# RyanXLi/OneshotDet

Hardware: AMD Instinct MI355X
Metric: images/sec/GPU fwd+bwd, 800x1024 target + 127x127 query, bs=8; 1->8 GPU scaling (higher is better)
Workload: dtype bf16; 1 GPU; BASELINE.json configs[2]: bs=8/GPU, 800x1024 target + 127x127 query, bf16 MFMA convs, forward (two R-50-FPN backbones, query pooling, correlation, FCOS head, training proposals) + FCOS loss + backward (stem/layer1 frozen) + gradient all-reduce + SGD(momentum) + weight repack; global_batch=8, parallelism=dp1: one rank, no collective anywhere in the step, world_size=1

## Files before the change

### oneshotdet_amd/_lib.py

```python
import ctypes as C
import os

_HERE = os.path.dirname(os.path.abspath(__file__))
LIB_PATH = os.environ.get("OSD_LIB_PATH") or os.path.join(_HERE, "lib", "liboneshotdet_hip.so")

OSD_F32, OSD_BF16 = 0, 1
ABI_VERSION = 4
ACT_NONE, ACT_RELU, ACT_EXP_SCALE = 0, 1, 2
RES_NONE, RES_SAME, RES_UP2X, RES_DOWN2X = 0, 1, 2, 3
GN_SPLITS = 64


class ConvDesc(C.Structure):
    _fields_ = [(n, C.c_int32) for n in (
        "dtype", "n", "h", "w", "cin", "in_stride_n", "in_stride_h", "in_stride_w", "ho", "wo", "cout", "r", "s",
        "stride_h", "stride_w", "pad_h", "pad_w", "w_rows", "out_stride", "res_mode", "res_h", "res_w", "res_stride",
        "act")] + [("act_scale", C.c_float), ("relu_in", C.c_int32), ("algo", C.c_int32), ("reserved0", C.c_int32),
                   ("ordered_ws", C.c_void_p), ("ordered_ws_bytes", C.c_int64)]


_p, _i, _f, _i64 = C.c_void_p, C.c_int, C.c_float, C.c_int64

SIGNATURES = {
    "osd_last_error_string": (C.c_char_p, []),
# ... 79 lines not shown
    "osd_box_decode": (_i, [_p, _p, _p, _p, _p, _p, _p, _i, _i, _i, _i, _p, _f, _f, _p, _f, _i, _p]),
    "osd_append_gt_boxes": (_i, [_p, _p, _p, _p, _p, _p, _p, _p, _i, _i, _i, _p]),
    "osd_proposals_sort_nms": (_i, [_p, _p, _i, _i, _i, _p, _p, _i, _i, _f, _i, _i, _p, _p, _p, _p, _p]),
    "osd_proposals_sort_nms_hint": (_i, [_p, _p, _i, _i, _i, _p, _p, _i, _i, _f, _i, _i, _i, _p, _p, _p, _p, _p, _p]),
    "osd_proposals_workspace_bytes": (_i64, [_i, _i, _i, _i]),
    "osd_box_match_sample": (_i, [_p, _p, _p, _p, _p, _p, _i, _i, _i, _i, _f, _f, _p, _p, _p, _p, _p, _p, _p, _p, _p]),
    "osd_box_loss": (_i, [_p, _p, _p, _p, _i, _i, _i, _f, _f, _p, _p, _i, _i, _p]),
    "osd_voc_match": (_i, [_p, _p, _p, _p, _p, _p, _p, _p, _i, _i, _i, _f, _p, _p, _p]),
    "osd_voc_curves": (_i, [_p, _p, _p, _i, _p, _p, _p]),
    "osd_voc_ap": (_i, [_p, _p, _p, _p, _p, _i, _i, _p, _p]),
    "osd_coco_match": (_i, [_p, _p, _p, _p, _p, _p, _i, _i, _i, _p, _i, _p, _i, _p, _p, _p, _p]),
    "osd_groupnorm_act_rois_bwd": (_i, [_p, _p, _p, _p, _p, _p, _p, _p, _p, _i, _i, _i, _i, _f, _f, _i, _i, _i, _i, _p]),
    "osd_rois_sum": (_i, [_p, _p, _i, _i, _i64, _i, _p]),
    "osd_roi_pool_levels_bwd": (_i, [_i, _p, _p, _p, _p, _p, _p, _p, _i, _i, _i, _i, _i, _i, _i, _p]),
    "osd_image_transform": (_i, [_p, _i, _i, _i, _i, _i, _i, _p, _p, _p, _i, _i, _i, _i, _i, _i, _i, _p, _p]),
    "osd_image_transform_workspace_bytes": (_i64, [_i, _i, _i, _i]),
    "osd_image_transform_batch": (_i, [_i, _p, _p, _p, _p, _p, _p, _i, _p, _p, _p, _i, _i, _i, _i, _i, _i, _i, _p, _p]),
}

BOX_CLS_CE, BOX_CLS_FOCAL, BOX_CLS_MSE = 0, 1, 2
SIGNATURES_BOX_MODES = {
    "osd_box_loss_opt": (_i, [_p, _p, _p, _p, _i, _i, _i, _f, _f, _p, _p, _i, _i, _i, _f, _f, _p]),
    "osd_box_decode_opt": (_i, [_p, _p, _p, _p, _p, _p, _p, _i, _i, _i, _i, _p, _f, _f, _p, _f, _i, _i, _p]),
}

BOX_CLS_L1, BOX_CLS_CXE = 3, 4
SOFT_LABEL_DISCRETE, SOFT_LABEL_LINEAR, SOFT_LABEL_TRANS_LINEAR, SOFT_LABEL_TRANS_4TH_LINEAR = 0, 1, 2, 3
SIGNATURES_SOFT_LABELS = {
    "osd_box_match_sample_soft": (_i, [_p, _p, _p, _p, _p, _p, _i, _i, _i, _i, _f, _f, _p, _p, _p, _p, _p, _p, _p, _p, _i, _p, _p, _p]),
    "osd_box_loss_soft": (_i, [_p, _p, _p, _p, _i, _i, _i, _f, _f, _p, _p, _i, _i, _p, _i, _p]),
}

SIGNATURES_NEG_SUPPORT = {
    "osd_box_loss_neg_support": (_i, [_p, _p, _p, _p, _p, _i, _i, _i, _f, _f, _f, _f, _p, _p, _p, _i, _i, _p]),
}

SIGNATURES_SOLVER = {
    "osd_solver_set": (_i, [_p, _f, _i, _p]),
    "osd_sgd_momentum_multi_dev": (_i, [_p, _p, _i, _p, _p, _p, _p, _f, _p]),
    "osd_sgd_momentum_pack_multi_dev": (_i, [_p, _p, _i, _p, _p, _p, _p, _p, _i, _p, _f, _i, _p]),
}

SIGNATURES_CLASS_SWEEP = {
    "osd_class_sweep_group": (_i, []),
    "osd_correlate_levels_sweep": (_i, [_i, _p, _p, _p, _p, _i, _i, _i, _i, _p]),
    "osd_roi_pool_levels_sweep": (_i, [_i, _p, _p, _p, _p, _p, _p, _p, _i, _i, _i, _i, _i, _i, _i, _p, _i, _p]),
}

SIGNATURES_GALLERY = {
    "osd_correlate_levels_gallery": (_i, [_i, _p, _p, _p, _p, _p, _i, _i, _i, _i, _i, _p]),
    "osd_groupnorm_act_rois_gallery": (_i, [_p, _p, _p, _p, _p, _p, _i, _i, _i, _i, _f, _f, _i, _i, _i, _i, _i, _p]),
}

_lib = None


class OsdError(RuntimeError):
    pass


def load():
    global _lib
    if _lib is not None:
        return _lib
    if not os.path.exists(LIB_PATH):
        raise OsdError("liboneshotdet_hip.so not built (%s missing): run `python -m oneshotdet_amd.build` or "
                       "__graft_entry__.build(); there is no CPU/eager fallback" % LIB_PATH)
    import torch
    lib = C.CDLL(LIB_PATH)
    for name, (res, args) in (list(SIGNATURES.items()) + list(SIGNATURES_BOX_MODES.items()) + list(SIGNATURES_SOFT_LABELS.items())
                              + list(SIGNATURES_NEG_SUPPORT.items()) + list(SIGNATURES_SOLVER.items())
                              + list(SIGNATURES_CLASS_SWEEP.items()) + list(SIGNATURES_GALLERY.items())):
        fn = getattr(lib, name)
        fn.restype = res
        fn.argtypes = args
    if lib.osd_abi_version() != ABI_VERSION:
        raise OsdError("%s reports ABI %d, this binding is written for ABI %d: rebuild it (`python -m oneshotdet_amd.build`)"
                       % (LIB_PATH, lib.osd_abi_version(), ABI_VERSION))
    _lib = lib
    return lib


def check(rc, what=""):
    if rc != 0:
        msg = load().osd_last_error_string()
        err = OsdError("%s failed (%d): %s" % (what, rc, msg.decode() if msg else "?"))
        err.code = rc
        raise err


def call(name, *args):
    lib = load()
    check(getattr(lib, name)(*args), name)
```

### oneshotdet_amd/build.py

```python
import os
import subprocess
import sys

HERE = os.path.dirname(os.path.abspath(__file__))
CSRC = os.path.join(HERE, "csrc")
LIBDIR = os.path.join(HERE, "lib")
TAG = os.environ.get("OSD_BUILD_TAG", "")
LIB = os.path.join(LIBDIR, "liboneshotdet_hip%s.so" % ("_" + TAG if TAG else ""))
SOURCES = ["osd_error.hip", "conv_igemm.hip", "conv_igemm_dma.hip", "conv_igemm_sp.hip", "conv_pred.hip", "conv_px.hip", "conv_wgrad.hip", "conv_wgrad_sk.hip", "backward.hip", "groupnorm_onepass.hip", "loss.hip", "elementwise.hip", "proposals.hip", "box_head.hip", "transforms.hip", "box_train.hip", "evaluation.hip", "query_avgpool.hip", "class_sweep.hip", "gallery.hip"]
HIPCC = os.environ.get("HIPCC", "/opt/rocm/bin/hipcc")
FLAGS = ["--offload-arch=gfx950", "-O3", "-fPIC", "-std=c++17", "-Wno-unused-result"] + os.environ.get("OSD_BUILD_FLAGS", "").split()


def _stale(target, deps):
    if not os.path.exists(target):
        return True
    t = os.path.getmtime(target)
    return any(os.path.getmtime(d) > t for d in deps)


def build_library(force=False, verbose=True):
    os.makedirs(LIBDIR, exist_ok=True)
    objdir = os.path.join(LIBDIR, "obj" + ("_" + TAG if TAG else ""))
    os.makedirs(objdir, exist_ok=True)
    headers = sorted(os.path.join(CSRC, f) for f in os.listdir(CSRC) if f.endswith(".h")) + [os.path.join(os.path.dirname(HERE), "include", h) for h in ("oneshotdet_hip.h", "oneshotdet_hip_box_modes.h", "oneshotdet_hip_soft_labels.h", "oneshotdet_hip_neg_support.h", "oneshotdet_hip_solver.h", "oneshotdet_hip_class_sweep.h", "oneshotdet_hip_gallery.h")]
    keep = set(src.replace(".hip", ".o") for src in SOURCES)
    for f in os.listdir(objdir):
        if f.endswith(".o") and f not in keep:
            os.remove(os.path.join(objdir, f))
    objs, procs = [], []
    for src in SOURCES:
        s = os.path.join(CSRC, src)
        o = os.path.join(objdir, src.replace(".hip", ".o"))
        objs.append(o)
        if force or _stale(o, [s] + headers):
            cmd = [HIPCC] + FLAGS + ["-c", s, "-o", o]
            if verbose:
                print(" ".join(cmd), flush=True)
            procs.append((src, subprocess.Popen(cmd, stdout=subprocess.PIPE, stderr=subprocess.STDOUT)))
    for src, p in procs:
        out, _ = p.communicate()
        if p.returncode != 0:
            sys.stderr.write(out.decode())
            raise RuntimeError("hipcc failed on %s" % src)
    if force or procs or _stale(LIB, objs):
        cmd = [HIPCC, "--offload-arch=gfx950", "-shared", "-fPIC", "-o", LIB] + objs
        if verbose:
            print(" ".join(cmd), flush=True)
        subprocess.check_call(cmd)
    return LIB


if __name__ == "__main__":
    print(build_library(force="--force" in sys.argv))
```

### oneshotdet_amd/ops.py

```python
import ctypes as C
import os

import torch

from . import _lib, spec
from ._lib import (ACT_EXP_SCALE, ACT_NONE, ACT_RELU, GN_SPLITS, OSD_BF16, OSD_F32, RES_DOWN2X, RES_NONE, RES_SAME, RES_UP2X,
                   ConvDesc)

__all__ = ["ACT_NONE", "ACT_RELU", "ACT_EXP_SCALE", "RES_NONE", "RES_SAME", "RES_UP2X", "RES_DOWN2X"]


from . import streams

_stream_handle = streams.raw_handle


def _stream():
    return C.c_void_p(_stream_handle())


from .trace import rec as _rec


def _dt(t):
    if t.dtype == torch.float32:
        return OSD_F32
    if t.dtype == torch.bfloat16:
        return OSD_BF16
    raise TypeError("unsupported activation dtype %s" % t.dtype)


class _Ptr(C.c_void_p):
    """a device address that keeps its tensor alive: `_ptr(x.contiguous())` on a non-contiguous x creates a temporary whose block the
    caching allocator would hand to the NEXT allocation made while the argument list is still being built (before the launch)"""


def _ptr(t):
    if t is None:
        return C.c_void_p(0)
    p = _Ptr(t.data_ptr())
    p.keep = t
    return p


def _chk_dev(*ts):
    for t in ts:
        if t is not None and not t.is_cuda:
            raise _lib.OsdError("oneshotdet_amd ops need device tensors (no CPU path): got %s" % t.device)


def conv_out(n, k, s, p):
    return (n + 2 * p - k) // s + 1


class PackedConv(object):
    __slots__ = ("w", "bias", "cout", "cout_store", "w_rows", "cin_k", "cin_real", "r", "s", "stem")

    def __init__(self, w, bias, cout, cout_store, w_rows, cin_k, r, s, stem=False, cin_real=None):
        self.w, self.bias, self.cout, self.cout_store = w, bias, cout, cout_store
        self.w_rows, self.cin_k, self.r, self.s, self.stem = w_rows, cin_k, r, s, stem
        self.cin_real = cin_k if cin_real is None else cin_real


def _round_up(x, m):
    return (x + m - 1) // m * m


def pack_conv(weight, bias=None, bn=None, dtype=torch.float32, stem=False):
    _chk_dev(weight)
    cout, cin, r, s = weight.shape
    weight = weight.contiguous().float()
    scale = None
    if bn is not None:
        g, b, mean, var = (t.float() for t in bn)
# ... 669 lines not shown


def _wgrad_mode():
    return _stream_handle() in _WGRAD_WS


def conv2d_wgrad(x, dy, dw_packed, r, s, stride, pad, cout, scale=None, db=None, algo=None):
    _chk_dev(x, dy, dw_packed)
    d = _conv_desc(x.shape, _dt(x), cout, r, s, stride, pad, dy.shape[-1])
    assert (dy.shape[1], dy.shape[2]) == (d.ho, d.wo), (dy.shape, d.ho, d.wo)
    st = _stream()

    def launch(dw, dbias):
        _lib.call("osd_conv2d_wgrad", C.byref(d), _p(x), _p(dy), _p(scale), _p(dw), _p(dbias), st)
    key = (d.dtype, tuple(x.shape), cout, r, s, stride, pad, dy.shape[-1], db is not None, _wgrad_mode())
    if algo is None:
        algo = WGRAD_ALGO_CACHE.get(key)
    if algo is None:
        algo = _tune_wgrad(key, d, launch, dw_packed, db, [x.shape[2]]) if _TUNING[0] else 0
    d.algo = algo
    launch(dw_packed, db)
    _rec("wgrad", items=[dict(x=x, dy=dy, dw=dw_packed, scale=scale, db=db, r=r, s=s, stride=stride, pad=pad, cout=cout)], algo=algo, key=key)


PRED_G = 64


def pred_gemm_ok(cout, r, s, stride, pad, cin, n_levels):
    return cout <= 4 and (r, s, stride, pad) == (3, 3, 1, 1) and cin % 256 == 0 and n_levels <= 6


def pred_dy_gather(dys, cout, cin):
    dy0 = dys[0]
    d = _conv_desc((dy0.shape[0], dy0.shape[1], dy0.shape[2], cin), _dt(dy0), cout, 3, 3, 1, 1, dy0.shape[-1])
    k = len(dys)
    tot = sum(t.shape[0] * t.shape[1] * t.shape[2] for t in dys)
    g = torch.empty((tot, PRED_G), device=dy0.device, dtype=dy0.dtype)
    ptrs = (C.c_void_p * k)(*[t.data_ptr() for t in dys])
    ns = (C.c_int32 * k)(*[t.shape[0] for t in dys])
    hs = (C.c_int32 * k)(*[t.shape[1] for t in dys])
    ws = (C.c_int32 * k)(*[t.shape[2] for t in dys])
    _lib.call("osd_pred_dy_gather", C.byref(d), k, ptrs, ns, hs, ws, _p(g), _stream())
    _rec("pred_gather", dys=list(dys), cout=cout, out=g)
    return g


def pred_dgrad_pack(w_master, cout, cin, dtype, out=None):
    wd = torch.empty((cin, 1, 1, PRED_G), device=w_master.device, dtype=dtype) if out is None else out
    _lib.call("osd_pred_dgrad_pack", _dt(wd), _p(w_master), cout, cin, _p(wd), _stream())
    _rec("pred_dgrad_pack", w=w_master, cout=cout, cin=cin, out=wd)
    return wd


def conv2d_wgrad_grouped(pairs, dw_packed, r, s, stride, pad, cout, scale=None, db=None, algo=None, g=None):
    x0, dy0 = pairs[0]
    d = _conv_desc(x0.shape, _dt(x0), cout, r, s, stride, pad, dy0.shape[-1])
    k = len(pairs)
    xs = (C.c_void_p * k)(*[x.data_ptr() for x, _ in pairs])
    dys = (C.c_void_p * k)(*[dy.data_ptr() for _, dy in pairs])
    ns = (C.c_int32 * k)(*[x.shape[0] for x, _ in pairs])
    hs = (C.c_int32 * k)(*[x.shape[1] for x, _ in pairs])
    ws = (C.c_int32 * k)(*[x.shape[2] for x, _ in pairs])
    st = _stream()
    if (cout <= 4 and (r, s, stride, pad) == (3, 3, 1, 1) and x0.shape[-1] % 256 == 0 and scale is None and k <= 6
            and not os.environ.get("OSD_NO_PRED_WGRAD")):
        if g is not None and not os.environ.get("OSD_PRED_WGRAD_READONCE"):
            wsp = torch.empty((64 + PRED_G * x0.shape[-1] + 64,), device=x0.device, dtype=torch.float32)
            _lib.call("osd_conv2d_wgrad_pred_gathered", C.byref(d), k, xs, _p(g), ns, hs, ws, _p(dw_packed), _p(db), _p(wsp), st)
        else:
            need = int(_lib.load().osd_conv2d_wgrad_pred_workspace_bytes(k, ns, hs, ws, x0.shape[-1]))
            wsp = torch.empty((need // 4 + 1,), device=x0.device, dtype=torch.float32)
            _lib.call("osd_conv2d_wgrad_pred", C.byref(d), k, xs, dys, ns, hs, ws, _p(dw_packed), _p(db), _p(wsp), st)
        _rec("wgrad", items=[dict(x=x, dy=dy, dw=dw_packed, scale=None, db=db, r=r, s=s, stride=stride, pad=pad, cout=cout)
                             for x, dy in pairs], algo="pred", key=None)
        return

    def launch(dw, dbias):
        _lib.call("osd_conv2d_wgrad_grouped", C.byref(d), k, xs, dys, ns, hs, ws, _p(scale), _p(dw), _p(dbias), st)
    key = (d.dtype, tuple(tuple(x.shape) for x, _ in pairs), cout, r, s, stride, pad, dy0.shape[-1], db is not None, _wgrad_mode())
    if algo is None:
        algo = WGRAD_ALGO_CACHE.get(key)
    if algo is None:
        algo = _tune_wgrad(key, d, launch, dw_packed, db, [x.shape[2] for x, _ in pairs]) if _TUNING[0] else 0
    d.algo = algo
    launch(dw_packed, db)
    _rec("wgrad", items=[dict(x=x, dy=dy, dw=dw_packed, scale=scale, db=db, r=r, s=s, stride=stride, pad=pad, cout=cout)
                         for x, dy in pairs], algo=algo, key=key)


def conv2d_wgrad_batched(items, r, s, stride, pad, cout, algo=None):
    x0, dy0 = items[0][0], items[0][1]
    assert all(it[0].shape == x0.shape and it[1].shape == dy0.shape for it in items)
    d = _conv_desc(x0.shape, _dt(x0), cout, r, s, stride, pad, dy0.shape[-1])
    k = len(items)
    xs = (C.c_void_p * k)(*[it[0].data_ptr() for it in items])
    dys = (C.c_void_p * k)(*[it[1].data_ptr() for it in items])
    scales = (C.c_void_p * k)(*[(it[3].data_ptr() if it[3] is not None else 0) for it in items])
    st = _stream()
    has_db = any(it[4] is not None for it in items)

    def launch(dws, dbs):
        dwp = (C.c_void_p * k)(*[t.data_ptr() for t in dws])
        dbp = (C.c_void_p * k)(*[(t.data_ptr() if t is not None else 0) for t in dbs])
        _lib.call("osd_conv2d_wgrad_batched", C.byref(d), k, xs, dys, scales, dwp, dbp, st)
    key = ("batched", k, d.dtype, tuple(x0.shape), cout, r, s, stride, pad, dy0.shape[-1], has_db, _wgrad_mode())
    if algo is None:
# ... 569 lines not shown
```

### oneshotdet_amd/train.py

```python
import math
import os

import torch

from . import streams

from . import ops, spec

from .train_backward import BackwardPass
from .train_forward import SIZE_RANGES, ForwardPass
from .train_second_stage import SecondStage
from .train_state import State
from .train_update import Update


def _payload(t):
    from .layers import ImageList
    if isinstance(t, ops.PackedImages):
        return t.tensor
    if isinstance(t, ImageList):
        return t.tensors
    return t


# ... 44 lines not shown
        self.pg = process_group
        self.wstream = torch.cuda.Stream(device=self.device) if wgrad_side_stream else None
        self.s1 = torch.cuda.Stream(device=self.device) if wgrad_side_stream else None
        self.wstream2 = torch.cuda.Stream(device=self.device) if wgrad_side_stream else None
        self.pstream = torch.cuda.Stream(device=self.device) if wgrad_side_stream else None
        self._keep = []
        self.second_stage = bool(second_stage)
        self.box_keys, self.box_losses = None, None
        self.box_suppress_loss = None
        from .model import ProposalDepth
        self._prop_depth = None if os.environ.get("OSD_NO_PROP_HINT") else ProposalDepth()
        self.lockstep = os.environ.get("OSD_LOCKSTEP", "0") != "0"
        self.corr_levels = os.environ.get("OSD_CORR_LEVELS", "1") != "0"
        self.skip_unused_c2 = os.environ.get("OSD_FULL_C2", "0") == "0"
        self.towers_merged = os.environ.get("OSD_TOWERS_MERGED", "0") != "0"
        self.split_levels = os.environ.get("OSD_SPLIT_LEVELS", "0") != "0"
        self.fuse_head_sum = os.environ.get("OSD_NO_HEAD_SUM_FUSION", "0") == "0"
        if not self.siamese_backbone:
            self.BBS = ("backbone.", "backbone.")
        self._shared_held = {}
        sd = {k: torch.as_tensor(v).to(self.device, torch.float32) for k, v in state_dict.items()
              if self.siamese_backbone or not spec.is_query_backbone_key(k)}
        missing = [k for k in spec.hot_path_shapes(self.siamese_backbone) if k not in sd]
        if missing:
            raise KeyError("state_dict is missing hot-path keys (siamese_backbone=%r), e.g. %s" % (self.siamese_backbone, missing[:3]))
        self._frozen_sd = sd
        self.convs = {}
        self.extra = {}
        self._plan = []
        self._build(sd)
        self._allocate(sd)
        from . import model as _model
        self._fused_l1 = {}
        if _model.FUSE_DOWNSAMPLE and dtype == torch.bfloat16:
            for bb in dict.fromkeys(self.BBS):
                if (bb + "body.layer1.0.downsample.0.weight") in sd:
                    self._fused_l1[bb] = _model.pack_conv3_downsample(sd, bb + "body.layer1.0.", dtype)
        from .dist_utils import GradExchange, bucket_ranges
        self.ustream = torch.cuda.Stream(device=self.device)
        for pair in [a for a in os.environ.get("OSD_STREAM_ALIAS", "").split(",") if "=" in a]:
            names = {"w": "wstream", "w2": "wstream2", "s1": "s1", "p": "pstream", "u": "ustream"}
            dst, src = pair.split("=")
            if getattr(self, names[src]) is not None:
                setattr(self, names[dst], getattr(self, names[src]))
        self.exchange = GradExchange(self.flat_g, bucket_ranges(self._plan, self.flat_g.numel()), self.pg,
                                     single_rank_too=exchange_single_rank, wire_dtype=grad_wire_dtype, comm_stream=self.ustream)
        self._overlap, self._fuse_update, self._updated = True, False, set()
        self.consume_grads = os.environ.get("OSD_NO_CONSUME_GRADS", "0") == "0"
        self._grads_clean, self._zeroed = False, set()
        self._wqs = None
        self._pred_grad_bufs = {}
        self.pred_dgrad_gemm = os.environ.get("OSD_NO_PRED_DGRAD_GEMM", "0") == "0"
        self._pred_dgrad = {}
        self.tower_wgrad_at = os.environ.get("OSD_TOWER_WGRAD_AT", "")
        self._held_wgrads = []
        if ordered_wgrad is None:
            ordered_wgrad = os.environ.get("OSD_WGRAD_ORDERED", "0") != "0"
        self.ordered_wgrad = bool(ordered_wgrad)
        self.fuse_gn_bwd = (not self.ordered_wgrad and self.dtype == torch.bfloat16 and os.environ.get("OSD_GN_FUSION", "0") != "0")
        self._gnb_ws = {}
        self.fpn_out_grouped = os.environ.get("OSD_NO_FPN_GROUPED", "0") == "0"
        self.gn_conv_db = (not self.ordered_wgrad and os.environ.get("OSD_NO_GN_CONV_DB", "0") == "0" and not ops.GN_ONEPASS_BWD)
        self.fuse_gn_fwd = (not self.ordered_wgrad and self.dtype == torch.bfloat16 and os.environ.get("OSD_GN_FWD_FUSION", "0") != "0")
        self._gnf_ws = {}
        cands = (self.wstream, self.wstream2) + ((self.pstream,) if self.second_stage else ())
        self._wgrad_streams = list({id(x): x for x in cands if x is not None}.values()) or [streams.current()]
        if self.ordered_wgrad and self.second_stage:
            import warnings
            warnings.warn("ordered_wgrad makes every conv_wgrad launch bit-reproducible, the second stage's included; its "
                          "ROI-pool backward (osd_roi_pool_levels_bwd) still scatters with fp32 atomics, so the gradients it "
                          "feeds into both backbones are reproducible only up to the order of those adds")
        for st in self._wgrad_streams:
            ops.wgrad_set_workspace(st, (1 << 30) if self.ordered_wgrad else 0)
        if self.wstream is not None:
            self.warm_streams()
        self.defer_join = False
        self._deferred, self._defer_now, self._joined_refs = None, False, None
        self.repack()
        self.zero_bias = torch.zeros(4096, device=self.device, dtype=torch.float32)
        weights = [c.w for c in self.convs.values() if c.trainable] + \
                  [p for n, (p, _) in self.extra.items() if "bias" not in n]
        biases = [c.b for c in self.convs.values() if c.trainable and c.has_bias] + \
                 [p for n, (p, _) in self.extra.items() if "bias" in n]
        self.lr, self.momentum, self.weight_decay = lr, momentum, weight_decay
        self.lr_schedule, self._solver, self._dev_update = lr_schedule, None, False
        self.opt = None
        if optimizer == "torch":
            self.opt = torch.optim.SGD([{"params": weights, "lr": lr, "weight_decay": weight_decay},
                                        {"params": biases, "lr": 2 * lr, "weight_decay": 0.0}], lr=lr, momentum=momentum)
            self._sgd = dict(tables={}, buf=None, steps=0)
        else:
            self._build_sgd_table(weights, biases)

    def _add_conv(self, name, sd, bn=None, bias=None, trainable=True):
        w = sd[name + ".weight"]
        cout, cin, r, s = w.shape
        c = TConv(name, cout, cin, r, s, trainable, bias is not None)
        if bn is not None:
            g, b, mean, var = (sd[bn + k] for k in (".weight", ".bias", ".running_mean", ".running_var"))
            c.bn_scale = (g * var.rsqrt()).contiguous()
            c.bn_shift = (b - mean * c.bn_scale).contiguous()
        self.convs[name] = c
        if trainable:
            self._plan.append((name + ".weight", (cout, r, s, cin)))
            if bias is not None:
                self._plan.append((name + ".bias", (cout,)))
# ... 426 lines not shown
```

### oneshotdet_amd/train_backward.py

```python

import torch

from . import streams

from . import ops, spec


class BackwardPass(object):
    def _wstream_of(self, which):
        if self.wstream is None:
            return None
        return self.wstream2 if (which == 1 and self.wstream2 is not None) else self.wstream

    def _on_wstream(self, fn, tensors, which=0):
        ws = self._wstream_of(which)
        if ws is None:
            return fn()
        ev = torch.cuda.Event()
        ev.record()
        ws.wait_event(ev)
        with streams.on(ws):
            fn()
        self._keep.append(tensors)

# ... 4 lines not shown
        ws = self._wstream_of(which)
        producers = [cur if ws is None else ws] + list(extra)
        if self._fuse_update and cur not in producers:
            producers.append(cur)
        if self.exchange.active:
            self.exchange.ready(name, producers)
        if not self._fuse_update:
            return
        ust = self.exchange.comm if self.exchange.active else self.ustream
        if not self.exchange.active:
            for st in producers:
                ev = torch.cuda.Event()
                ev.record(st)
                ust.wait_event(ev)
        with streams.on(ust):
            self._update_bucket(name)

    def _flush_wgrads(self, j, which):
        q, self._wqs[j] = self._wqs[j], []
        for i in range(0, len(q), 24):
            part = q[i:i + 24]
            if len(part) == 1:
                c, x, dy, stride, pad = part[0]
                self._on_wstream(lambda c=c, x=x, dy=dy, stride=stride, pad=pad: ops.conv2d_wgrad(
                    x, dy, c.gw, c.r, c.s, stride, pad, c.cout, scale=c.bn_scale, db=c.gb if c.has_bias else None), (x, dy),
                    which)
            else:
                items = [(x, dy, c.gw, c.bn_scale, c.gb if c.has_bias else None, c.r, c.s, stride, pad, c.cout)
                         for c, x, dy, stride, pad in part]
                self._on_wstream(lambda items=items: ops.conv2d_wgrad_mixed(items), items, which)

    def _flush_shared_stage(self, sname, which0):
        q, self._wqs[0] = self._wqs[0], []
        if which0 == 1:
            ev = torch.cuda.Event()
            ev.record()
            self._shared_held[sname] = (q, ev)
            return False
        held = self._shared_held.pop(sname, None)
        if held is not None:
            ws = self._wstream_of(0) or streams.current()
            ws.wait_event(held[1])
            q = held[0] + q
        self._wqs[0] = q
        self._flush_wgrads(0, 0)
        return True

    def _wgrad_grouped(self, c, pairs, which=0, g=None):
        self._on_wstream(lambda: ops.conv2d_wgrad_grouped(pairs, c.gw, c.r, c.s, 1, c.r // 2, c.cout, scale=c.bn_scale,
                                                          db=c.gb if c.has_bias else None, g=g), (pairs, g), which)

    def _pred_backward(self, c, t_last, dpred, which):
        nl = len(dpred)
        g = ops.pred_dy_gather(dpred, c.cout, c.cin)
        self._wgrad_grouped(c, [(t_last[l], dpred[l]) for l in range(nl)], which, g=g)
        ent = self.pred_dgrad_weights(c, fresh_ok=True)
        dx = ops.conv2d(g.view(1, 1, g.shape[0], ops.PRED_G), ent)
        out, q0 = [], 0
        for t in dpred:
            n, hh, ww = t.shape[0], t.shape[1], t.shape[2]
            out.append(dx.view(-1, c.cin)[q0:q0 + n * hh * ww].view(n, hh, ww, c.cin))
            q0 += n * hh * ww
        return out

    def pred_dgrad_weights(self, c, fresh_ok=False):
        key = ("pred_dgrad", c.name)
        ent = self._pred_dgrad.get(key)
        if ent is None:
            wd = torch.empty((c.cin, 1, 1, ops.PRED_G), device=self.device, dtype=self.dtype)
            ent = self._pred_dgrad[key] = ops.PackedConv(wd, torch.zeros(ops._round_up(c.cin, 16), device=self.device, dtype=torch.float32),
                                                         c.cin, c.cin, c.cin, ops.PRED_G, 1, 1, cin_real=9 * c.cout)
        fresh = getattr(self, "_pred_dgrad_fresh", None)
        if fresh is None:
            fresh = self._pred_dgrad_fresh = set()
        if fresh_ok and c.name in fresh:
            fresh.discard(c.name)
            return ent
        ops.pred_dgrad_pack(c.w, c.cout, c.cin, self.dtype, out=ent.w)
        if not fresh_ok:
            fresh.add(c.name)
        return ent

    def _dgrad_levels(self, c, dys):
        return ops.conv2d_grouped(dys, c.pd, pad=c.r - 1 - (c.r // 2))

    def head_backward(self, feats, ctxs, pred_grads):
        nl = len(feats)
        if self.towers_merged:
            d_t = self._towers_backward(ctxs, pred_grads, self.TOWERS, nl)
        else:
            main = streams.current()
            side = self.s1 if self.s1 is not None else main
            side.wait_stream(main)
            with streams.on(side):
                d_t = self._towers_backward(ctxs, pred_grads, ("bbox_tower",), nl)
            if self.fuse_head_sum:
                def bbox_grads():
                    main.wait_stream(side)
                    self._keep.append(d_t["bbox_tower"])
                    return d_t["bbox_tower"]
                return self._towers_backward(ctxs, pred_grads, ("cls_tower",), nl, last_addends=bbox_grads)["cls_tower"]
            d_t.update(self._towers_backward(ctxs, pred_grads, ("cls_tower",), nl))
            main.wait_stream(side)
        return [ops.add_mask(d_t["cls_tower"][l], d_t["bbox_tower"][l]) for l in range(nl)]

    def _towers_backward(self, ctxs, pred_grads, towers, nl, last_addends=None):
# ... 192 lines not shown
```

Baseline: 784.7 images/sec.

## Fuse prediction-conv dgrad and wgrad into a single gather+MFMA backward kernel

Adds a HIP kernel that gathers the im2col'd dy for the small-cout 3x3 prediction convs once into LDS. It then computes both dx (via packed transposed weights) and per-workgroup partial dw/db with MFMA, followed by a reduction kernel. This replaces the separate dy-gather, grouped wgrad launch and dgrad GEMM, removing repeated reads of dy and x and several launches. The trade-off is that wgrad now runs on the main stream instead of the side wgrad stream, which loses that overlap, and it adds a partial-sum workspace.

```diff
diff --git a/include/oneshotdet_hip_pred_bwd.h b/include/oneshotdet_hip_pred_bwd.h
--- /dev/null
+++ b/include/oneshotdet_hip_pred_bwd.h
@@ -0,0 +1,24 @@
+#ifndef ONESHOTDET_HIP_PRED_BWD_H
+#define ONESHOTDET_HIP_PRED_BWD_H
+
+#include "oneshotdet_hip.h"
+
+#ifdef __cplusplus
+extern "C" {
+#endif
+
+#define OSD_PRED_BWD_BOTH 0
+#define OSD_PRED_BWD_DGRAD 1
+#define OSD_PRED_BWD_WGRAD 2
+
+int64_t osd_pred_bwd_workspace_bytes(int n_seg, const int32_t* ns, const int32_t* hs, const int32_t* ws, int cin, int cout);
+
+int osd_conv2d_pred_bwd(const osd_conv_desc* desc, int n_seg, const void* const* xs, const void* const* dys, const int32_t* ns,
+                        const int32_t* hs, const int32_t* ws, const void* wd_packed, void* dx, float* dw, float* db, void* workspace,
+                        int flags, void* stream);
+
+#ifdef __cplusplus
+}
+#endif
+
+#endif
diff --git a/oneshotdet_amd/_lib.py b/oneshotdet_amd/_lib.py
--- a/oneshotdet_amd/_lib.py
+++ b/oneshotdet_amd/_lib.py
@@ -155,6 +155,12 @@
     "osd_groupnorm_act_rois_gallery": (_i, [_p, _p, _p, _p, _p, _p, _i, _i, _i, _i, _f, _f, _i, _i, _i, _i, _i, _p]),
 }
 
+PRED_BWD_BOTH, PRED_BWD_DGRAD, PRED_BWD_WGRAD = 0, 1, 2
+SIGNATURES_PRED_BWD = {
+    "osd_pred_bwd_workspace_bytes": (_i64, [_i, _p, _p, _p, _i, _i]),
+    "osd_conv2d_pred_bwd": (_i, [C.POINTER(ConvDesc), _i, _p, _p, _p, _p, _p, _p, _p, _p, _p, _p, _i, _p]),
+}
+
 _lib = None
 
 
@@ -173,7 +179,8 @@
     lib = C.CDLL(LIB_PATH)
     for name, (res, args) in (list(SIGNATURES.items()) + list(SIGNATURES_BOX_MODES.items()) + list(SIGNATURES_SOFT_LABELS.items())
                               + list(SIGNATURES_NEG_SUPPORT.items()) + list(SIGNATURES_SOLVER.items())
-                              + list(SIGNATURES_CLASS_SWEEP.items()) + list(SIGNATURES_GALLERY.items())):
+                              + list(SIGNATURES_CLASS_SWEEP.items()) + list(SIGNATURES_GALLERY.items())
+                              + list(SIGNATURES_PRED_BWD.items())):
         fn = getattr(lib, name)
         fn.restype = res
         fn.argtypes = args
diff --git a/oneshotdet_amd/build.py b/oneshotdet_amd/build.py
--- a/oneshotdet_amd/build.py
+++ b/oneshotdet_amd/build.py
@@ -7,7 +7,7 @@
 LIBDIR = os.path.join(HERE, "lib")
 TAG = os.environ.get("OSD_BUILD_TAG", "")
 LIB = os.path.join(LIBDIR, "liboneshotdet_hip%s.so" % ("_" + TAG if TAG else ""))
-SOURCES = ["osd_error.hip", "conv_igemm.hip", "conv_igemm_dma.hip", "conv_igemm_sp.hip", "conv_pred.hip", "conv_px.hip", "conv_wgrad.hip", "conv_wgrad_sk.hip", "backward.hip", "groupnorm_onepass.hip", "loss.hip", "elementwise.hip", "proposals.hip", "box_head.hip", "transforms.hip", "box_train.hip", "evaluation.hip", "query_avgpool.hip", "class_sweep.hip", "gallery.hip"]
+SOURCES = ["osd_error.hip", "conv_igemm.hip", "conv_igemm_dma.hip", "conv_igemm_sp.hip", "conv_pred.hip", "conv_pred_bwd.hip", "conv_px.hip", "conv_wgrad.hip", "conv_wgrad_sk.hip", "backward.hip", "groupnorm_onepass.hip", "loss.hip", "elementwise.hip", "proposals.hip", "box_head.hip", "transforms.hip", "box_train.hip", "evaluation.hip", "query_avgpool.hip", "class_sweep.hip", "gallery.hip"]
 HIPCC = os.environ.get("HIPCC", "/opt/rocm/bin/hipcc")
 FLAGS = ["--offload-arch=gfx950", "-O3", "-fPIC", "-std=c++17", "-Wno-unused-result"] + os.environ.get("OSD_BUILD_FLAGS", "").split()
 
@@ -23,7 +23,7 @@
     os.makedirs(LIBDIR, exist_ok=True)
     objdir = os.path.join(LIBDIR, "obj" + ("_" + TAG if TAG else ""))
     os.makedirs(objdir, exist_ok=True)
-    headers = sorted(os.path.join(CSRC, f) for f in os.listdir(CSRC) if f.endswith(".h")) + [os.path.join(os.path.dirname(HERE), "include", h) for h in ("oneshotdet_hip.h", "oneshotdet_hip_box_modes.h", "oneshotdet_hip_soft_labels.h", "oneshotdet_hip_neg_support.h", "oneshotdet_hip_solver.h", "oneshotdet_hip_class_sweep.h", "oneshotdet_hip_gallery.h")]
+    headers = sorted(os.path.join(CSRC, f) for f in os.listdir(CSRC) if f.endswith(".h")) + [os.path.join(os.path.dirname(HERE), "include", h) for h in ("oneshotdet_hip.h", "oneshotdet_hip_box_modes.h", "oneshotdet_hip_soft_labels.h", "oneshotdet_hip_neg_support.h", "oneshotdet_hip_solver.h", "oneshotdet_hip_class_sweep.h", "oneshotdet_hip_gallery.h", "oneshotdet_hip_pred_bwd.h")]
     keep = set(src.replace(".hip", ".o") for src in SOURCES)
     for f in os.listdir(objdir):
         if f.endswith(".o") and f not in keep:
diff --git a/oneshotdet_amd/csrc/conv_pred_bwd.hip b/oneshotdet_amd/csrc/conv_pred_bwd.hip
--- /dev/null
+++ b/oneshotdet_amd/csrc/conv_pred_bwd.hip
@@ -0,0 +1,347 @@
+#include "osd_common.h"
+#include "../../include/oneshotdet_hip_pred_bwd.h"
+
+#include <stdlib.h>
+
+#define OSD_STREAM(s) reinterpret_cast<hipStream_t>(s)
+
+namespace {
+
+constexpr int kLevels = 6;
+constexpr int kG = 64;
+constexpr int TP = 128;
+constexpr int SP = 64;
+
+struct PredBwdLevels {
+  const void* x[kLevels];
+  const void* dy[kLevels];
+  int H[kLevels], W[kLevels], npix[kLevels], begin[kLevels];
+  int n_levels;
+};
+
+__device__ __attribute__((aligned(16))) unsigned g_pb_zero[4];
+
+typedef __attribute__((address_space(3))) bf16x4* lds_bf4_ptr;
+
+__device__ __forceinline__ int pb_swz(int row) { return ((row >> 1) & 3) << 1; }
+__device__ __forceinline__ int pb_off(int row, int chunk) { return row * 128 + ((chunk ^ pb_swz(row)) << 4); }
+
+template <bool DG, bool WG>
+__global__ void __launch_bounds__(256, 2) pred_bwd_kernel(PredBwdLevels L, const __bf16* __restrict__ wd, __bf16* __restrict__ dx,
+                                                          float* __restrict__ part, float* __restrict__ part_b, int cin, int cout,
+                                                          int dy_stride, int tot, int ppw) {
+  __shared__ __attribute__((aligned(16))) char s_g[TP * 128];
+  __shared__ __attribute__((aligned(16))) char s_x[4 * SP * 128];
+  __shared__ const char* s_row[TP];
+  __shared__ float s_b[4][4];
+
+  const int tid = threadIdx.x, lane = tid & 63;
+  const int wave = __builtin_amdgcn_readfirstlane(tid >> 6);
+  const int cg = blockIdx.y;
+  const int p0 = blockIdx.x * ppw, p1 = min(tot, p0 + ppw);
+  const int g4 = lane >> 4, l16 = lane & 15;
+
+  bf16x8 wa[4][2];
+  if constexpr (DG) {
+#pragma unroll
+    for (int i = 0; i < 4; ++i) {
+      const int ci = cg * 256 + wave * 64 + (i >> 1) * 32 + (l16 >> 2) * 8 + (i & 1) * 4 + (l16 & 3);
+#pragma unroll
+      for (int ks = 0; ks < 2; ++ks) wa[i][ks] = *reinterpret_cast<const bf16x8*>(wd + (size_t)ci * kG + ks * 32 + g4 * 8);
+    }
+  }
+  f32x4 acc[3][4];
+#pragma unroll
+  for (int i = 0; i < 3; ++i)
+#pragma unroll
+    for (int j = 0; j < 4; ++j) acc[i][j] = f32x4{0.f, 0.f, 0.f, 0.f};
+  float bsum[4] = {0.f, 0.f, 0.f, 0.f};
+
+  char* sx = s_x + wave * (SP * 128);
+  bf16x8 xr[8];
+  auto load_stage = [&](int s) {
+#pragma unroll
+    for (int i = 0; i < 8; ++i) {
+      const char* rp = s_row[s * SP + i * 8 + (lane >> 3)];
+      const char* src = rp != nullptr ? rp + wave * 128 + (lane & 7) * 16 : reinterpret_cast<const char*>(g_pb_zero);
+      xr[i] = *reinterpret_cast<const bf16x8*>(src);
+    }
+  };
+
+  for (int t0 = p0; t0 < p1; t0 += TP) {
+    const int rows = min(TP, p1 - t0);
+    __syncthreads();
+#pragma unroll
+    for (int it = 0; it < TP * 8 / 256; ++it) {
+      const int idx = it * 256 + tid;
+      const int px = idx >> 3, c8 = idx & 7;
+      const bool valid = px < rows;
+      const int q_all = valid ? t0 + px : p0;
+      int lvl = 0;
+#pragma unroll
+      for (int i = 1; i < kLevels; ++i)
+        if (i < L.n_levels && q_all >= L.begin[i]) lvl = i;
+      const void* dyv = L.dy[0];
+      const void* xv = L.x[0];
+      int H = L.H[0], W = L.W[0], beg = L.begin[0];
+#pragma unroll
+      for (int i = 1; i < kLevels; ++i)
+        if (lvl == i) { dyv = L.dy[i]; xv = L.x[i]; H = L.H[i]; W = L.W[i]; beg = L.begin[i]; }
+      const __bf16* __restrict__ dy = reinterpret_cast<const __bf16*>(dyv);
+      const int q = q_all - beg, HW = H * W;
+      const int img = q / HW, rem = q - img * HW, qy = rem / W, qx = rem - qy * W;
+      bf16x8 out;
+#pragma unroll
+      for (int h = 0; h < 2; ++h) {
+        const int t = 2 * c8 + h;
+        const int py = qy - t / 3 + 1, pxx = qx - t % 3 + 1;
+        const bool ok = valid && t < 9 && (unsigned)py < (unsigned)H && (unsigned)pxx < (unsigned)W;
+        const bf16x4* src = ok ? reinterpret_cast<const bf16x4*>(dy + ((size_t)(img * H + py) * W + pxx) * dy_stride)
+                               : reinterpret_cast<const bf16x4*>(g_pb_zero);
+        const bf16x4 v = *src;
+#pragma unroll
+        for (int co = 0; co < 4; ++co) out[h * 4 + co] = co < cout ? v[co] : (__bf16)0.f;
+      }
+      if (c8 == 2) {
+#pragma unroll
+        for (int co = 0; co < 4; ++co) bsum[co] += (float)out[co];
+      }
+      *reinterpret_cast<bf16x8*>(s_g + pb_off(px, c8)) = out;
+      if (c8 == 0)
+        s_row[px] = valid ? reinterpret_cast<const char*>(xv) + ((size_t)q * cin + cg * 256) * 2 : nullptr;
+    }
+    __syncthreads();
+    const int nst = (rows + SP - 1) / SP;
+    if constexpr (WG) load_stage(0);
+
+    if constexpr (DG) {
+      for (int n = 0; n * 16 < rows; ++n) {
+        const int row = n * 16 + l16;
+        const bf16x8 b0 = *reinterpret_cast<const bf16x8*>(s_g + pb_off(row, g4));
+        const bf16x8 b1 = *reinterpret_cast<const bf16x8*>(s_g + pb_off(row, 4 + g4));
+        f32x4 d[4];
+#pragma unroll
+        for (int i = 0; i < 4; ++i) {
+          d[i] = __builtin_amdgcn_mfma_f32_16x16x32_bf16(wa[i][0], b0, f32x4{0.f, 0.f, 0.f, 0.f}, 0, 0, 0);
+          d[i] = __builtin_amdgcn_mfma_f32_16x16x32_bf16(wa[i][1], b1, d[i], 0, 0, 0);
+        }
+        if (row < rows) {
+          __bf16* o = dx + (size_t)(t0 + row) * cin + cg * 256 + wave * 64 + g4 * 8;
+#pragma unroll
+          for (int h = 0; h < 2; ++h) {
+            bf16x8 v;
+#pragma unroll
+            for (int e = 0; e < 4; ++e) { v[e] = (__bf16)d[2 * h][e]; v[4 + e] = (__bf16)d[2 * h + 1][e]; }
+            *reinterpret_cast<bf16x8*>(o + h * 32) = v;
+          }
+        }
+      }
+    }
+
+    if constexpr (WG) {
+#pragma unroll
+      for (int s = 0; s < TP / SP; ++s) {
+        if (s < nst) {
+          __builtin_amdgcn_fence(__ATOMIC_ACQ_REL, "wavefront");
+#pragma unroll
+          for (int i = 0; i < 8; ++i) *reinterpret_cast<bf16x8*>(sx + pb_off(i * 8 + (lane >> 3), lane & 7)) = xr[i];
+          if (s + 1 < nst) load_stage(s + 1);
+          __builtin_amdgcn_fence(__ATOMIC_ACQ_REL, "wavefront");
+          __builtin_amdgcn_wave_barrier();
+          const int q4 = l16 >> 2, pp = l16 & 3, h8 = (pp & 1) * 8;
+#pragma unroll
+          for (int kk = 0; kk < SP / 32; ++kk) {
+            if (s * SP + kk * 32 < rows) {
+              const int rs1 = kk * 32 + 4 * g4 + q4, rs2 = rs1 + 16;
+              const int rg1 = s * SP + rs1, rg2 = rg1 + 16;
+              bf16x8 af[3], bfr[4];
+#pragma unroll
+              for (int i = 0; i < 3; ++i) {
+                const int chunk = 2 * i + (pp >> 1);
+                const bf16x4 lo = __builtin_amdgcn_ds_read_tr16_b64_v4bf16((lds_bf4_ptr)(s_g + pb_off(rg1, chunk) + h8));
+                const bf16x4 hi = __builtin_amdgcn_ds_read_tr16_b64_v4bf16((lds_bf4_ptr)(s_g + pb_off(rg2, chunk) + h8));
+#pragma unroll
+                for (int e = 0; e < 4; ++e) { af[i][e] = lo[e]; af[i][e + 4] = hi[e]; }
+              }
+#pragma unroll
+              for (int j = 0; j < 4; ++j) {
+                const int chunk = 2 * j + (pp >> 1);
+                const bf16x4 lo = __builtin_amdgcn_ds_read_tr16_b64_v4bf16((lds_bf4_ptr)(sx + pb_off(rs1, chunk) + h8));
+                const bf16x4 hi = __builtin_amdgcn_ds_read_tr16_b64_v4bf16((lds_bf4_ptr)(sx + pb_off(rs2, chunk) + h8));
+#pragma unroll
+                for (int e = 0; e < 4; ++e) { bfr[j][e] = lo[e]; bfr[j][e + 4] = hi[e]; }
+              }
+#pragma unroll
+              for (int i = 0; i < 3; ++i)
+#pragma unroll
+                for (int j = 0; j < 4; ++j) acc[i][j] = __builtin_amdgcn_mfma_f32_16x16x32_bf16(af[i], bfr[j], acc[i][j], 0, 0, 0);
+            }
+          }
+        }
+      }
+    }
+  }
+
+  if constexpr (WG) {
+    const int rows_real = 9 * cout;
+    float* pp = part + ((size_t)blockIdx.x * gridDim.y + cg) * rows_real * 256 + wave * 64 + l16;
+#pragma unroll
+    for (int i = 0; i < 3; ++i)
+#pragma unroll
+      for (int e = 0; e < 4; ++e) {
+        const int grow = 16 * i + 4 * g4 + e, tap = grow >> 2, co = grow & 3;
+        if (tap < 9 && co < cout) {
+#pragma unroll
+          for (int j = 0; j < 4; ++j) pp[(co * 9 + tap) * 256 + 16 * j] = acc[i][j][e];
+        }
+      }
+    if (cg == 0) {
+#pragma unroll
+      for (int co = 0; co < 4; ++co) {
+        float v = bsum[co];
+#pragma unroll
+        for (int m = 32; m >= 1; m >>= 1) v += __shfl_xor(v, m, 64);
+        if (lane == 0) s_b[wave][co] = v;
+      }
+      __syncthreads();
+      if (tid < 4) part_b[(size_t)blockIdx.x * 4 + tid] = (s_b[0][tid] + s_b[1][tid]) + (s_b[2][tid] + s_b[3][tid]);
+    }
+  }
+}
+
+__global__ void __launch_bounds__(256) pred_bwd_reduce_kernel(const float* __restrict__ part, const float* __restrict__ part_b,
+                                                              float* __restrict__ dw, float* __restrict__ db, int nwg, int groups,
+                                                              int cin, int cout) {
+  __shared__ float s[16][17];
+  const int e = threadIdx.x & 15, sl = threadIdx.x >> 4;
+  const int n = cout * 9 * cin;
+  const bool bias = (int)blockIdx.x == n / 16;
+  const int per = (nwg + 15) / 16;
+  const int b0 = sl * per, b1 = min(nwg, b0 + per);
+  const int i = blockIdx.x * 16 + e;
+  const float* p;
+  size_t stride;
+  bool on;
+  if (!bias) {
+    const int ci = i % cin, ct = i / cin;
+    p = part + ((size_t)(ci >> 8) * 9 * cout + ct) * 256 + (ci & 255);
+    stride = (size_t)groups * 9 * cout * 256;
+    on = true;
+  } else {
+    p = part_b + e;
+    stride = 4;
+    on = e < cout;
+  }
+  float a[16];
+#pragma unroll
+  for (int u = 0; u < 16; ++u) a[u] = 0.f;
+  if (on) {
+    for (int b = b0; b < b1; b += 16) {
+      float v[16];
+#pragma unroll
+      for (int u = 0; u < 16; ++u) {
+        const bool ok = b + u < b1;
+        v[u] = p[(size_t)(ok ? b + u : b0) * stride];
+        if (!ok) v[u] = 0.f;
+      }
+#pragma unroll
+      for (int u = 0; u < 16; ++u) a[u] += v[u];
+    }
+  }
+  s[sl][e] = (((a[0] + a[1]) + (a[2] + a[3])) + ((a[4] + a[5]) + (a[6] + a[7]))) + (((a[8] + a[9]) + (a[10] + a[11])) + ((a[12] + a[13]) + (a[14] + a[15])));
+  __syncthreads();
+  if (sl == 0 && on) {
+    float t = 0.f;
+#pragma unroll
+    for (int k = 0; k < 16; ++k) t += s[k][e];
+    if (!bias) dw[i] += t;
+    else db[e] += t;
+  }
+}
+
+void pred_bwd_plan(long long tot, int groups, int* ppw, int* nwg) {
+  static int target = -1;
+  if (target < 0) { const char* e = getenv("OSD_PRED_BWD_WGS"); target = e ? atoi(e) : 0; if (target < 1) target = 512; }
+  int t = target / groups;
+  if (t < 1) t = 1;
+  long long p = ((tot + t - 1) / t + 15) / 16 * 16;
+  if (p < 272) p = 272;
+  *ppw = (int)p;
+  *nwg = (int)((tot + p - 1) / p);
+}
+
+int pred_bwd_check(const osd_conv_desc* d, int n_seg, const int32_t* ns, const int32_t* hs, const int32_t* ws, long long* tot_out) {
+  if (!d || !ns || !hs || !ws || n_seg < 1 || n_seg > kLevels) return osd_fail(OSD_ERR_INVALID_ARG, "pred_bwd: bad arguments (1..%d levels)", kLevels);
+  if (d->dtype != OSD_F32 && d->dtype != OSD_BF16) return osd_fail(OSD_ERR_INVALID_ARG, "pred_bwd: bad dtype");
+  if (d->dtype != OSD_BF16) return osd_fail(OSD_ERR_UNSUPPORTED, "pred_bwd: bf16 only");
+  if (d->cout < 1 || d->cout > 4 || d->r != 3 || d->s != 3 || d->stride_h != 1 || d->stride_w != 1 || d->pad_h != 1 || d->pad_w != 1 ||
+      d->cin <= 0 || d->cin % 256 != 0 || d->out_stride < 4 || d->out_stride % 4 != 0)
+    return osd_fail(OSD_ERR_UNSUPPORTED, "pred_bwd: 3x3 / stride 1 / pad 1, cout <= 4, cin %% 256 == 0, dy rows of >= 4 channels");
+  long long tot = 0;
+  for (int i = 0; i < n_seg; ++i) {
+    if (ns[i] <= 0 || hs[i] <= 0 || ws[i] <= 0) return osd_fail(OSD_ERR_INVALID_ARG, "pred_bwd: bad segment %d", i);
+    const long long npix = (long long)ns[i] * hs[i] * ws[i];
+    if (npix > 0x7fffffffLL / d->out_stride) return osd_fail(OSD_ERR_INVALID_ARG, "pred_bwd: bad segment %d", i);
+    tot += npix;
+  }
+  if (tot > 0x7fffffffLL / 8) return osd_fail(OSD_ERR_INVALID_ARG, "pred_bwd: too many pixels");
+  *tot_out = tot;
+  return OSD_OK;
+}
+
+}
+
+extern "C" int64_t osd_pred_bwd_workspace_bytes(int n_seg, const int32_t* ns, const int32_t* hs, const int32_t* ws, int cin, int cout) {
+  if (n_seg < 1 || n_seg > kLevels || !ns || !hs || !ws || cin <= 0 || cin % 256 != 0 || cout < 1 || cout > 4) return 0;
+  long long tot = 0;
+  for (int i = 0; i < n_seg; ++i) tot += (long long)ns[i] * hs[i] * ws[i];
+  if (tot <= 0) return 0;
+  int ppw, nwg;
+  pred_bwd_plan(tot, cin / 256, &ppw, &nwg);
+  return (int64_t)nwg * (cin / 256) * 9 * cout * 256 * 4 + (int64_t)nwg * 4 * 4 + 256;
+}
+
+extern "C" int osd_conv2d_pred_bwd(const osd_conv_desc* d, int n_seg, const void* const* xs, const void* const* dys, const int32_t* ns,
+                                   const int32_t* hs, const int32_t* ws, const void* wd_packed, void* dx, float* dw, float* db,
+                                   void* workspace, int flags, void* stream) {
+  long long tot = 0;
+  int rc = pred_bwd_check(d, n_seg, ns, hs, ws, &tot);
+  if (rc) return rc;
+  if (flags != OSD_PRED_BWD_BOTH && flags != OSD_PRED_BWD_DGRAD && flags != OSD_PRED_BWD_WGRAD)
+    return osd_fail(OSD_ERR_INVALID_ARG, "pred_bwd: bad flags %d", flags);
+  const bool dg = flags != OSD_PRED_BWD_WGRAD, wg = flags != OSD_PRED_BWD_DGRAD;
+  if (!dys || (wg && (!xs || !dw || !workspace)) || (dg && (!wd_packed || !dx))) return osd_fail(OSD_ERR_INVALID_ARG, "pred_bwd: null argument");
+  if (((size_t)wd_packed | (size_t)dx | (size_t)workspace) & 15) return osd_fail(OSD_ERR_INVALID_ARG, "pred_bwd: wd_packed, dx and workspace must be 16-byte aligned");
+  PredBwdLevels L;
+  L.n_levels = n_seg;
+  long long beg = 0;
+  for (int i = 0; i < kLevels; ++i) {
+    const int j = i < n_seg ? i : 0;
+    if (!dys[j] || (wg && !xs[j])) return osd_fail(OSD_ERR_INVALID_ARG, "pred_bwd: null segment %d", j);
+    if (((size_t)dys[j] & 7) || (wg && ((size_t)xs[j] & 15))) return osd_fail(OSD_ERR_INVALID_ARG, "pred_bwd: segment %d: dy must be 8-byte, x 16-byte aligned", j);
+    const long long npix = (long long)ns[j] * hs[j] * ws[j];
+    L.x[i] = wg ? xs[j] : nullptr; L.dy[i] = dys[j]; L.H[i] = hs[j]; L.W[i] = ws[j];
+    L.npix[i] = i < n_seg ? (int)npix : 0; L.begin[i] = i < n_seg ? (int)beg : 0x7fffffff;
+    if (i < n_seg) beg += npix;
+  }
+  const int groups = d->cin / 256;
+  int ppw, nwg;
+  pred_bwd_plan(tot, groups, &ppw, &nwg);
+  float* part = static_cast<float*>(workspace);
+  float* part_b = wg ? part + (size_t)nwg * groups * 9 * d->cout * 256 : nullptr;
+  hipStream_t st = OSD_STREAM(stream);
+  const dim3 grid(nwg, groups);
+#define OSD_PB_LAUNCH(DG, WG)                                                                                                        \
+  hipLaunchKernelGGL((pred_bwd_kernel<DG, WG>), grid, dim3(256), 0, st, L, (const __bf16*)wd_packed, (__bf16*)dx, part, part_b, d->cin, \
+                     d->cout, d->out_stride, (int)tot, ppw)
+  if (dg && wg) OSD_PB_LAUNCH(true, true);
+  else if (dg) OSD_PB_LAUNCH(true, false);
+  else OSD_PB_LAUNCH(false, true);
+#undef OSD_PB_LAUNCH
+  rc = osd_check_launch("pred_bwd");
+  if (rc || !wg) return rc;
+  const int n = d->cout * 9 * d->cin;
+  hipLaunchKernelGGL(pred_bwd_reduce_kernel, dim3(n / 16 + (db ? 1 : 0)), dim3(256), 0, st, (const float*)part, (const float*)part_b, dw, db,
+                     nwg, groups, d->cin, d->cout);
+  return osd_check_launch("pred_bwd(reduce)");
+}
diff --git a/oneshotdet_amd/ops.py b/oneshotdet_amd/ops.py
--- a/oneshotdet_amd/ops.py
+++ b/oneshotdet_amd/ops.py
@@ -20,6 +20,7 @@
 
 
 from .trace import rec as _rec
+from . import trace as _trace
 
 
 def _dt(t):
@@ -795,6 +796,48 @@
     return wd
 
 
+def pred_bwd_fused_ok(dtype, cout, r, s, stride, pad, cin, n_levels):
+    return dtype == torch.bfloat16 and pred_gemm_ok(cout, r, s, stride, pad, cin, n_levels)
+
+
+def pred_bwd_fused(xs, dys, wd_ent, dw, db, cout, flags=_lib.PRED_BWD_BOTH):
+    x0, dy0 = xs[0], dys[0]
+    _chk_dev(x0, dy0, dw)
+    cin = x0.shape[-1]
+    d = _conv_desc(x0.shape, _dt(x0), cout, 3, 3, 1, 1, dy0.shape[-1])
+    k = len(xs)
+    tot = sum(t.shape[0] * t.shape[1] * t.shape[2] for t in dys)
+    dg, wg = flags != _lib.PRED_BWD_WGRAD, flags != _lib.PRED_BWD_DGRAD
+    xp = (C.c_void_p * k)(*[t.data_ptr() for t in xs])
+    dyp = (C.c_void_p * k)(*[t.data_ptr() for t in dys])
+    ns = (C.c_int32 * k)(*[t.shape[0] for t in dys])
+    hs = (C.c_int32 * k)(*[t.shape[1] for t in dys])
+    ws = (C.c_int32 * k)(*[t.shape[2] for t in dys])
+    dx = torch.empty((tot, cin), device=x0.device, dtype=x0.dtype) if dg else None
+    wsp = None
+    if wg:
+        need = int(_lib.load().osd_pred_bwd_workspace_bytes(k, ns, hs, ws, cin, cout))
+        wsp = torch.empty((need // 4 + 1,), device=x0.device, dtype=torch.float32)
+    _lib.call("osd_conv2d_pred_bwd", C.byref(d), k, xp, dyp, ns, hs, ws, _p(wd_ent.w) if dg else None, _p(dx), _p(dw) if wg else None,
+              _p(db) if wg else None, _p(wsp), flags, _stream())
+    if wg:
+        _rec("wgrad", items=[dict(x=x, dy=dy, dw=dw, scale=None, db=db, r=3, s=3, stride=1, pad=1, cout=cout) for x, dy in zip(xs, dys)],
+             algo="pred", key=None)
+    if not dg:
+        return None
+    if _trace.TRACE is not None and not _TUNING[0]:
+        g = pred_dy_gather(dys, cout, cin)
+        _rec("conv", x=g.view(1, 1, tot, PRED_G), w=wd_ent.w, bias=wd_ent.bias, cout=wd_ent.cout_store, r=1, s=1, stem=False, stride=1,
+             pad=0, act=ACT_NONE, res=None, res_mode=RES_NONE, relu_in=False, act_scale=1.0, act_scale_dev=None, mask=None,
+             out=dx.view(1, 1, tot, cin), algo="pred_bwd", key=None)
+    out, q0 = [], 0
+    for t in dys:
+        n, hh, ww = t.shape[0], t.shape[1], t.shape[2]
+        out.append(dx[q0:q0 + n * hh * ww].view(n, hh, ww, cin))
+        q0 += n * hh * ww
+    return out
+
+
 def conv2d_wgrad_grouped(pairs, dw_packed, r, s, stride, pad, cout, scale=None, db=None, algo=None, g=None):
     x0, dy0 = pairs[0]
     d = _conv_desc(x0.shape, _dt(x0), cout, r, s, stride, pad, dy0.shape[-1])
diff --git a/oneshotdet_amd/train.py b/oneshotdet_amd/train.py
--- a/oneshotdet_amd/train.py
+++ b/oneshotdet_amd/train.py
@@ -120,6 +120,7 @@
         self._pred_grad_bufs = {}
         self.pred_dgrad_gemm = os.environ.get("OSD_NO_PRED_DGRAD_GEMM", "0") == "0"
         self._pred_dgrad = {}
+        self.pred_bwd_fused = os.environ.get("OSD_PRED_BWD_FUSED", "1") != "0"
         self.tower_wgrad_at = os.environ.get("OSD_TOWER_WGRAD_AT", "")
         self._held_wgrads = []
         if ordered_wgrad is None:
diff --git a/oneshotdet_amd/train_backward.py b/oneshotdet_amd/train_backward.py
--- a/oneshotdet_amd/train_backward.py
+++ b/oneshotdet_amd/train_backward.py
@@ -80,6 +80,9 @@
 
     def _pred_backward(self, c, t_last, dpred, which):
         nl = len(dpred)
+        if self.pred_bwd_fused and ops.pred_bwd_fused_ok(self.dtype, c.cout, c.r, c.s, 1, c.r // 2, c.cin, nl):
+            ent = self.pred_dgrad_weights(c, fresh_ok=True)
+            return ops.pred_bwd_fused(t_last, dpred, ent, c.gw, c.gb if c.has_bias else None, c.cout)
         g = ops.pred_dy_gather(dpred, c.cout, c.cin)
         self._wgrad_grouped(c, [(t_last[l], dpred[l]) for l in range(nl)], which, g=g)
         ent = self.pred_dgrad_weights(c, fresh_ok=True)
```

Result: faster. 792.9 images/sec, median of 6 (+1.0%).
